# google-research/nerf-from-image

Measured on AMD Instinct MI355X. Metric: rendered rays/sec (128x128, 64+64 samples), higher is better.
Workload: dtype f32 (decoder MLP operands split-fp16 hi+lo, 22 bits; strict fp32: config.value_mlp_exact_fp32)

## Files before the change

### nerf_from_image_amd/csrc/nfi_kernels.hip

```cpp
#include "nfi_device.hpp"
#include "../../include/nfi_hip.h"
#include "nfi_host.hpp"

#include <algorithm>
#include <cstdio>
#include <cstring>

using namespace nfi;

thread_local char nfi_err_buf[256] = "";
extern "C" const char* nfi_last_error(void) { return nfi_err_buf; }
extern "C" int nfi_version(void) { return 100; }


constexpr int kP2tPixels = 256, kP2tPitch = 288;
template <int TEX>
__global__ __launch_bounds__(256) void planes_to_texels_kernel(const float* __restrict__ planes, void* __restrict__ texels,
                                                               int hw) {
  __shared__ __attribute__((aligned(16))) float tile[kC][kP2tPitch];
  const int img = blockIdx.y;
  const int px0 = blockIdx.x * kP2tPixels;
  const float* src = planes + (size_t)img * kC * hw;
  {
    const int c4 = threadIdx.x & 63, r0 = threadIdx.x >> 6;
// ... 166 lines not shown
          w2v[h] = w;
        }
      }
      auto hi = __builtin_amdgcn_cvt_pkrtz(w2v[0], w2v[1]);
      auto lo = __builtin_amdgcn_cvt_pkrtz(w2v[0] - (float)hi[0], w2v[1] - (float)hi[1]);
      v = bits2f(hl == 0 ? __builtin_bit_cast(uint32_t, hi) : __builtin_bit_cast(uint32_t, lo));
    }
    image[i] = v;
  }
}

extern "C" size_t nfi_decoder_image_floats(void) { return (size_t)kImageFloats; }

extern "C" int nfi_decoder_pack(const float* w1, const float* b1, const float* w2, const float* b2, int n_attention,
                                int texel_dtype, float* image, nfi_stream_t stream) {
  REQUIRE(w1 && b1 && w2 && b2 && image, "decoder_pack: null pointer");
  REQUIRE(n_attention >= 0 && n_attention <= NFI_MAX_ATTENTION, "decoder_pack: attention_values must be in [0,14]");
  REQUIRE(texel_dtype >= NFI_TEXEL_F32 && texel_dtype <= NFI_TEXEL_F16, "decoder_pack: bad texel dtype");
  int n_out = n_attention > 0 ? 1 + n_attention : 4;
  hipLaunchKernelGGL(decoder_pack_kernel, dim3((kImageFloats + 255) / 256), dim3(256), 0, (hipStream_t)stream, w1, b1, w2, b2,
                     n_out, texel_dtype, image);
  return check_launch("decoder_pack");
}

__global__ __launch_bounds__(256) void decoder_pack_vd_kernel(const float* __restrict__ w1, const float* __restrict__ b1,
                                                              const float* __restrict__ w2, const float* __restrict__ b2,
                                                              const float* __restrict__ w3, const float* __restrict__ b3,
                                                              int n3, int tex, float* __restrict__ image) {
  const float gain1 = 0.17677669529663687f;
  const float gain2 = 0.125f;
  const float gain3 = 0.17677669529663687f;
  for (int i = threadIdx.x; i < kVdImageFloats; i += blockDim.x) {
    float v = 0.0f;
    if (i < kVdB1F) {
      int k = i - kVdW1F;
      int nt = k & 3, lane = (k >> 2) & 63, s = k >> 8;
      int row = 16 * nt + (lane & 15);
      int ch = feat_channel(tex, s, lane >> 4);
      v = (w1[row * kC + ch] * gain1) * (kLog2e / 3.0f);
    } else if (i < kVdW2) {
      int k = i - kVdB1F;
      int r = k & 3, nt = (k >> 2) & 3, g = k >> 4;
      v = b1[16 * nt + 4 * g + r] * kLog2e;
    } else if (i < kVdB2) {
      int k = i - kVdW2;
      int r = k & 3, lane = (k >> 2) & 63, nt = (k >> 8) & 3, t = k >> 10;
      int row = 16 * t + (lane & 15);
      int hid = 16 * nt + 4 * (lane >> 4) + r;
      if (row < 33) v = (w2[row * kHidden + hid] * gain2) * kLn2;
    } else if (i < kVdW3) {
      int row = i - kVdB2;
      if (row < 33) v = b2[row];
    } else if (i < kVdB3) {
      int k = i - kVdW3;
      int r = k & 3, lane = (k >> 2) & 63, t = k >> 8;
      int out = lane & 15;
      int kk = 16 * t + 4 * (lane >> 4) + r;
      if (out == 0) v = (kk == 0) ? 1.0f : 0.0f;
      else if (out <= n3 && kk >= 1 && kk <= 32) v = (w3[(out - 1) * 32 + (kk - 1)] * gain3) * kLog2e;
    } else {
      int out = i - kVdB3;
      if (out >= 1 && out <= n3) v = b3[out - 1] * kLog2e;
    }
    image[i] = v;
  }
}

extern "C" size_t nfi_decoder_image_floats_viewdir(void) { return (size_t)kVdImageFloats; }

extern "C" int nfi_decoder_pack_viewdir(const float* w1, const float* b1, const float* w2, const float* b2, const float* w3,
                                        const float* b3, int n_attention, int texel_dtype, float* image,
                                        nfi_stream_t stream) {
  REQUIRE(w1 && b1 && w2 && b2 && w3 && b3 && image, "decoder_pack_viewdir: null pointer");
  REQUIRE(n_attention >= 0 && n_attention <= NFI_MAX_ATTENTION, "decoder_pack_viewdir: attention_values must be in [0,14]");
  REQUIRE(texel_dtype >= NFI_TEXEL_F32 && texel_dtype <= NFI_TEXEL_F16, "decoder_pack_viewdir: bad texel dtype");
  static_assert(NFI_RAY_FEATURE_PITCH == kRayFeatPad, "ray feature pitch");
  int n3 = n_attention > 0 ? n_attention : 3;
  hipLaunchKernelGGL(decoder_pack_vd_kernel, dim3(1), dim3(256), 0, (hipStream_t)stream, w1, b1, w2, b2, w3, b3, n3,
                     texel_dtype, image);
  return check_launch("decoder_pack_viewdir");
}

constexpr int kRayBlocks = 256;
__device__ __forceinline__ void block_reduce_keys(uint32_t kmin, uint32_t kmax, uint32_t cnt, uint32_t* reduce) {
  __shared__ uint32_t s_min[4], s_max[4], s_cnt[4];
#pragma unroll
  for (int d = 32; d >= 1; d >>= 1) {
    uint32_t a = (uint32_t)__shfl_xor((int)kmin, d, 64), b = (uint32_t)__shfl_xor((int)kmax, d, 64);
    kmin = a > kmin ? a : kmin;
    kmax = b > kmax ? b : kmax;
    cnt += (uint32_t)__shfl_xor((int)cnt, d, 64);
  }
  int wave = threadIdx.x >> 6;
  if ((threadIdx.x & 63) == 0) { s_min[wave] = kmin; s_max[wave] = kmax; s_cnt[wave] = cnt; }
  __syncthreads();
  if (threadIdx.x == 0) {
    int nw = blockDim.x >> 6;
    for (int w = 1; w < nw; ++w) {
      kmin = s_min[w] > kmin ? s_min[w] : kmin;
      kmax = s_max[w] > kmax ? s_max[w] : kmax;
      cnt += s_cnt[w];
    }
    if (cnt) {
      atomicMax(&reduce[0], kmin);
      atomicMax(&reduce[1], kmax);
      atomicAdd(&reduce[2], cnt);
    }
  }
}

struct RaygenOut {
  float* ro; float* rd;
  float* near_raw; float* far_raw; uint8_t* hit;
  uint32_t* reduce;
  float scene_range;
};

__global__ __launch_bounds__(256) void raygen_kernel(CameraParams cam, int n_scenes, RaygenOut out) {
  const int hw = cam.rows * cam.width;
  const int64_t n = (int64_t)n_scenes * hw;
  uint32_t kmin = 0u, kmax = 0u, cnt = 0u;
  for (int64_t ray = (int64_t)blockIdx.x * blockDim.x + threadIdx.x; ray < n; ray += (int64_t)gridDim.x * blockDim.x) {
    int b = (int)(ray / hw);
    int pix = (int)(ray - (int64_t)b * hw);
    int row = pix / cam.width, col = pix - row * cam.width;
    float o[3], d[3];
    make_ray(cam, b, cam.row0 + row, col, o, d);
    if (out.ro) { out.ro[ray * 3 + 0] = o[0]; out.ro[ray * 3 + 1] = o[1]; out.ro[ray * 3 + 2] = o[2]; }
    if (out.rd) { out.rd[ray * 3 + 0] = d[0]; out.rd[ray * 3 + 1] = d[1]; out.rd[ray * 3 + 2] = d[2]; }
    if (out.near_raw) {
      float near = 0.0f, far = 0.0f;
      const bool hit = slab_test(o, d, out.scene_range, near, far);
      float n2, f2;
      bool hit_wide = slab_test(o, d, out.scene_range * 1.0001f, n2, f2);
      out.near_raw[ray] = near;
      out.far_raw[ray] = far;
      out.hit[ray] = (uint8_t)((hit ? 1 : 0) | (hit_wide ? 2 : 0));
      if (hit) {
        const uint32_t a = ~ordered_key(near), c = ordered_key(far);
        kmin = a > kmin ? a : kmin;
        kmax = c > kmax ? c : kmax;
        ++cnt;
      }
    }
  }
  if (out.near_raw) block_reduce_keys(kmin, kmax, cnt, out.reduce);
}

__global__ __launch_bounds__(256) void slab_kernel(const float* __restrict__ ro, const float* __restrict__ rd, int64_t n,
                                                   float scene_range, float* __restrict__ near_raw,
                                                   float* __restrict__ far_raw, uint8_t* __restrict__ hit_out,
                                                   uint32_t* reduce) {
  uint32_t kmin = 0u, kmax = 0u, cnt = 0u;
  for (int64_t ray = (int64_t)blockIdx.x * blockDim.x + threadIdx.x; ray < n; ray += (int64_t)gridDim.x * blockDim.x) {
    float o[3] = {ro[ray * 3], ro[ray * 3 + 1], ro[ray * 3 + 2]};
    float d[3] = {rd[ray * 3], rd[ray * 3 + 1], rd[ray * 3 + 2]};
    float near = 0.0f, far = 0.0f;
    const bool hit = slab_test(o, d, scene_range, near, far);
    float n2, f2;
    bool hit_wide = slab_test(o, d, scene_range * 1.0001f, n2, f2);
    near_raw[ray] = near;
    far_raw[ray] = far;
    hit_out[ray] = (uint8_t)((hit ? 1 : 0) | (hit_wide ? 2 : 0));
    if (hit) {
      const uint32_t a = ~ordered_key(near), c = ordered_key(far);
      kmin = a > kmin ? a : kmin;
      kmax = c > kmax ? c : kmax;
      ++cnt;
    }
  }
  block_reduce_keys(kmin, kmax, cnt, reduce);
}

__global__ __launch_bounds__(256) void finish_planes_kernel(const float* __restrict__ near_raw,
                                                            const float* __restrict__ far_raw,
                                                            const uint8_t* __restrict__ hit, const uint32_t* __restrict__ reduce,
                                                            int64_t n, float* __restrict__ near_plane,
                                                            float* __restrict__ far_plane) {
  const int64_t ray = (int64_t)blockIdx.x * blockDim.x + threadIdx.x;
  if (ray >= n) return;
  float fill_near = ordered_key_inv(~reduce[0]), fill_far = ordered_key_inv(reduce[1]);
  float a = near_raw[ray], b = far_raw[ray];
  finish_planes((hit[ray] & 1) != 0, fill_near, fill_far, a, b);
  near_plane[ray] = a;
  far_plane[ray] = b;
}

extern "C" int nfi_raygen(const nfi_raygen_args* a, nfi_stream_t stream) {
  REQUIRE(a && a->cam2world && a->ray_origins && a->ray_directions, "raygen: null pointer");
  REQUIRE(a->n_scenes > 0 && a->height > 0 && a->width > 0, "raygen: bad shape");
  CameraParams cam{a->cam2world, a->focal, a->bbox, a->focal ? a->center : nullptr, a->height, a->width, a->normalize, a->height, 0};
  RaygenOut out{a->ray_origins, a->ray_directions, nullptr, nullptr, nullptr, nullptr, 0.0f};
  int64_t n = (int64_t)a->n_scenes * a->height * a->width;
  hipLaunchKernelGGL(raygen_kernel, dim3((unsigned)std::min<int64_t>((n + 255) / 256, kRayBlocks)), dim3(256), 0, (hipStream_t)stream, cam,
                     a->n_scenes, out);
  return check_launch("raygen");
}

extern "C" int nfi_near_far(const nfi_near_far_args* a, nfi_stream_t stream) {
  REQUIRE(a && a->ray_origins && a->ray_directions && a->near_raw && a->far_raw && a->hit && a->reduce,
          "near_far: null pointer");
  REQUIRE(a->n_rays > 0, "near_far: no rays");
  hipStream_t s = (hipStream_t)stream;
  if (hipMemsetAsync(a->reduce, 0, 16, s) != hipSuccess) return fail(NFI_ERR_LAUNCH, "near_far: memset failed");
  unsigned blocks = (unsigned)((a->n_rays + 255) / 256);
  hipLaunchKernelGGL(slab_kernel, dim3(std::min<unsigned>(blocks, kRayBlocks)), dim3(256), 0, s, a->ray_origins, a->ray_directions, a->n_rays,
                     a->scene_range, a->near_raw, a->far_raw, a->hit, a->reduce);
  if (a->near_plane && a->far_plane)
    hipLaunchKernelGGL(finish_planes_kernel, dim3(blocks), dim3(256), 0, s, a->near_raw, a->far_raw, a->hit, a->reduce,
                       a->n_rays, a->near_plane, a->far_plane);
  return check_launch("near_far");
}

__device__ __forceinline__ float stratified_depth(float near, float far, int k, int S, float noise, bool jitter) {
  float t = aten_lerp(near, far, (float)k / (float)S);
  if (jitter) t = t + noise * ((far - near) / (float)S);
  return t;
}

__global__ __launch_bounds__(256) void stratified_kernel(nfi_stratified_args a) {
  const int64_t idx = (int64_t)blockIdx.x * blockDim.x + threadIdx.x;
  const int64_t total = a.n_rays * a.n_samples;
  if (idx >= total) return;
  const int64_t ray = idx / a.n_samples;
  const int k = (int)(idx - ray * a.n_samples);
  float near = a.near_plane[ray], far = a.far_plane[ray];
  float t = stratified_depth(near, far, k, a.n_samples, a.noise ? a.noise[idx] : 0.0f, a.noise != nullptr);
  a.depth[idx] = t;
  if (a.points) {
#pragma unroll
    for (int c = 0; c < 3; ++c) a.points[idx * 3 + c] = a.ray_origins[ray * 3 + c] + a.ray_directions[ray * 3 + c] * t;
  }
}

__global__ __launch_bounds__(256) void points_on_rays_kernel(const float* __restrict__ ro, const float* __restrict__ rd,
                                                             const float* __restrict__ depth, int64_t total, int S,
                                                             float* __restrict__ points) {
  const int64_t idx = (int64_t)blockIdx.x * blockDim.x + threadIdx.x;
  if (idx >= total) return;
  const int64_t ray = idx / S;
  const float t = depth[idx];
#pragma unroll
  for (int c = 0; c < 3; ++c) points[idx * 3 + c] = ro[ray * 3 + c] + rd[ray * 3 + c] * t;
}

extern "C" int nfi_points_on_rays(const float* ray_origins, const float* ray_directions, const float* depth,
                                  int64_t n_rays, int n_samples, float* points, nfi_stream_t stream) {
  REQUIRE(ray_origins && ray_directions && depth && points, "points_on_rays: null pointer");
  REQUIRE(n_rays > 0 && n_samples > 0, "points_on_rays: bad shape");
  int64_t total = n_rays * n_samples;
  hipLaunchKernelGGL(points_on_rays_kernel, dim3((unsigned)((total + 255) / 256)), dim3(256), 0, (hipStream_t)stream,
                     ray_origins, ray_directions, depth, total, n_samples, points);
  return check_launch("points_on_rays");
}
// ... 721 lines not shown
    }
  }
  if (a.n_extra > 0 && a.extra_map) {
    wave_lds_fence();
#pragma unroll
    for (int j = 0; j < NS; ++j) {
      int e = j * 64 + lane;
      if (e < n) slab.cdf[e] = w[j];
    }
    wave_lds_fence();
    float we[NS];
#pragma unroll
    for (int j = 0; j < NS; ++j) { int e = j * 64 + lane; we[j] = e < n ? slab.cdf[rank[j]] : 0.0f; }
    for (int c = 0; c < a.n_extra; ++c) {
      float acc = 0.0f;
#pragma unroll
      for (int j = 0; j < NS; ++j) {
        int e = j * 64 + lane;
        if (e < na) acc += we[j] * a.extra_a[((size_t)ray * na + e) * a.n_extra + c];
        else if (e < n) acc += we[j] * a.extra_b[((size_t)ray * nb + (e - na)) * a.n_extra + c];
      }
      acc = wave_sum(acc);
      if (lane == 0) a.extra_map[ray * a.n_extra + c] = acc;
    }
  }
}

extern "C" int nfi_composite_fwd(const nfi_composite_args* a, nfi_stream_t stream) {
  REQUIRE(a && a->ray_directions && a->depth_a && a->sigma_a && a->rgb_a && a->rgb_map && a->depth_map && a->mask,
          "composite: null pointer");
  REQUIRE(a->n_rays > 0 && a->n_a > 0 && a->n_b >= 0 && a->n_a + a->n_b <= NFI_MAX_SAMPLES_SINGLE_PASS,
          "composite: need 1 <= n_a + n_b <= 512");
  REQUIRE(a->n_b == 0 || (a->n_a <= NFI_MAX_SAMPLES && a->n_b <= NFI_MAX_SAMPLES), "composite: merged lists hold at most 128 samples each");
  REQUIRE(a->n_b == 0 || (a->depth_b && a->sigma_b && a->rgb_b), "composite: list b missing");
  REQUIRE(a->n_extra == 0 || (a->extra_a && (a->n_b == 0 || a->extra_b)), "composite: extra attribute missing");
  const dim3 grid((unsigned)((a->n_rays + 3) / 4));
  if (a->n_a + a->n_b <= 128) hipLaunchKernelGGL(composite_kernel<2>, grid, dim3(256), 0, (hipStream_t)stream, *a);
  else if (a->n_a + a->n_b <= 256) hipLaunchKernelGGL(composite_kernel<4>, grid, dim3(256), 0, (hipStream_t)stream, *a);
  else hipLaunchKernelGGL(composite_kernel<8>, grid, dim3(256), 0, (hipStream_t)stream, *a);
  return check_launch("composite_fwd");
}

#include "nfi_backward_rays.inc"
#include "nfi_regulariser.inc"
#include "nfi_neighbours.inc"
#include "nfi_handoff.inc"
#include "nfi_pnp.inc"

struct RenderKernelParams {
  int n_scenes, hw, S;
  int fine, white;
  float scene_range;
  const float* ro; const float* rd; const float* near_raw; const float* far_raw; const uint8_t* hit;
  const uint32_t* reduce;
  uint32_t* counter;
  int width;
  int tile_order;
  int xcd_blocks;
  uint32_t* xcd_counter;
  int xcd_block_shift;
  int fetch_batch;
  const void* texels; int res; int layout;
  const float* image; int A; const float* att;
  int use_sdf; const float* beta; const float* alpha;
  const float* noise_c; const float* noise_f; int64_t noise_f_stride;
  float* rgb; float* depth; float* mask;
  float* near_plane; float* far_plane;
  float* t_coarse; float* sigma_coarse; float* rgb_coarse;
  float* t_fine; float* sigma_fine; float* rgb_fine;
  float* t_sorted; float* weights; int32_t* perm;
  int skip_missed;
  unsigned long long* prof;
  const float* xray;
  float term_eps;
  float* semantics;
  float* coords;
  float* normals;
  unsigned long long* clock_probe;
  FastDiv div_hw, div_bps, div_bw;
  int tap_stride;
  int stash;
};

struct ClockProbe {
  unsigned long long c0 = 0, r0 = 0;
  bool on = false;
  __device__ __forceinline__ void start(const RenderKernelParams& k) {
    on = k.clock_probe && blockIdx.x == 0 && threadIdx.x == 0;
    if (on) { c0 = __builtin_readcyclecounter(); r0 = __builtin_amdgcn_s_memrealtime(); }
  }
  __device__ __forceinline__ void stop(const RenderKernelParams& k) const {
    if (on) {
      k.clock_probe[0] = __builtin_readcyclecounter() - c0;
      k.clock_probe[1] = __builtin_amdgcn_s_memrealtime() - r0;
    }
  }
};

__device__ __forceinline__ float uniform_f32(float v) {
  return bits2f((uint32_t)__builtin_amdgcn_readfirstlane((int)f2bits(v)));
}

struct RayInputs {
  float ox, oy, oz, dx, dy, dz, near, far, noise, u;
  uint32_t hit;
};

struct RayQueue {
  const RenderKernelParams& k;
  int lane;
  uint32_t n_rays, xcd, bsh, bw, bps, n_blocks, q_cur, pos_next, pos_end, batch;
  bool dry;
  __device__ __forceinline__ RayQueue(const RenderKernelParams& kk, int l) : k(kk), lane(l) {
    n_rays = (uint32_t)k.n_scenes * (uint32_t)k.hw;
    xcd = k.xcd_blocks ? (__builtin_amdgcn_s_getreg(6164) & 7u) : 0u;
    bsh = (uint32_t)k.xcd_block_shift;
    bw = (uint32_t)k.width >> bsh;
    bps = bw * (((uint32_t)k.hw / (uint32_t)k.width) >> bsh);
    n_blocks = bps * (uint32_t)k.n_scenes;
    q_cur = xcd; pos_next = 0; pos_end = 0; dry = false;
    batch = (uint32_t)k.fetch_batch;
  }
  __device__ __forceinline__ uint32_t ray_at(uint32_t q, uint32_t pos) const {
    const uint32_t b = (pos >> (2 * bsh)) * 8u + q;
    const uint32_t in = pos & ((1u << (2 * bsh)) - 1u), scene = fastdiv(b, k.div_bps), bb = b - scene * bps;
    const uint32_t by = fastdiv(bb, k.div_bw), bx = bb - by * bw;
    const uint32_t st = in >> 6, sty = st >> (bsh - 3), stx = st & ((1u << (bsh - 3)) - 1u);
    const uint32_t y = (by << bsh) + (sty << 3) + ((in >> 3) & 7u), x = (bx << bsh) + (stx << 3) + (in & 7u);
    return scene * (uint32_t)k.hw + y * (uint32_t)k.width + x;
  }
  __device__ __forceinline__ uint32_t fetch() {
    if (!k.xcd_blocks) {
      uint32_t p = 0;
      if (lane == 0) p = atomicAdd(k.counter, 1u);
      return (uint32_t)__builtin_amdgcn_readfirstlane((int)p);
    }
    if (pos_next == pos_end && !dry) {
      dry = true;
      for (uint32_t i = 0; i < 8; ++i) {
        uint32_t base = 0;
        if (lane == 0) base = atomicAdd(k.xcd_counter + q_cur * 16, batch);
        base = (uint32_t)__builtin_amdgcn_readfirstlane((int)base);
        if ((base >> (2 * bsh)) * 8u + q_cur < n_blocks) { pos_next = base; pos_end = base + batch; dry = false; break; }
        q_cur = (q_cur + 1) & 7u;
      }
    }
    if (dry) return n_rays;
    return ray_at(q_cur, pos_next++);
  }
};

constexpr int kRenderPlain = 0, kRenderTaps = 1, kRenderProf = 2, kRenderTerm = 3, kRenderExtra = 4, kRenderNormals = 5;
constexpr int kSemPitch = 2 * 64 + 4;
constexpr int kSemPitchWide = 2 * 128 + 8;
extern __shared__ __attribute__((aligned(16))) float nfi_dyn_lds[];

typedef __attribute__((address_space(3))) float lds_float;

template <int NS, class Slab>
__device__ __forceinline__ void composite_coords(const Slab& slab, const float (&w)[NS], int n, int lane, float ox, float oy,
                                                 float oz, float dx, float dy, float dz, float* out3) {
  float cx = 0.0f, cy = 0.0f, cz = 0.0f;
#pragma unroll
  for (int j = 0; j < NS; ++j) {
    const int e = j * 64 + lane;
    if (e < n) {
      const float t = slab.srt[0][e];
      cx += w[j] * (ox + dx * t); cy += w[j] * (oy + dy * t); cz += w[j] * (oz + dz * t);
    }
  }
  cx = wave_sum(cx); cy = wave_sum(cy); cz = wave_sum(cz);
  if (lane == 0) { out3[0] = cx; out3[1] = cy; out3[2] = cz; }
}

template <int TEX, bool ATT, int OCC, int MODE, int PREC, bool VD = false>
__global__ __launch_bounds__(256, OCC) void render_fwd_kernel(RenderKernelParams k) {
  constexpr bool TAPS = MODE == kRenderTaps, PROF = MODE == kRenderProf, TERM = MODE == kRenderTerm;
  constexpr bool EXTRA = MODE == kRenderExtra || MODE == kRenderNormals, NRM = MODE == kRenderNormals;
  constexpr int SEMP = (EXTRA && ATT) ? kSemPitch : 0;
  constexpr int kImg = VD ? kVdImageFloats : kLdsImageFloats;
  __shared__ __attribute__((aligned(16))) float lds[kImg];
  __shared__ __attribute__((aligned(16))) float vfs[4][64];
  __shared__ WaveSlab slabs[4];
  if constexpr (NRM) stage_normal_operands(nfi_dyn_lds, k.image, VD ? kVdW1F : kW1F, VD ? kVdW2 : kW2F);
  ClockProbe clock;
  clock.start(k);
  if (PREC == 1) {
    for (int i = threadIdx.x; i < kB1F; i += blockDim.x) lds[i] = k.image[kW1H + i];
    for (int i = kB1F + threadIdx.x; i < kLdsImageFloats; i += blockDim.x) lds[i] = k.image[i];
  } else {
    for (int i = threadIdx.x; i < kImg; i += blockDim.x) lds[i] = k.image[i];
  }
  __syncthreads();
  const int lane = lane_id();
  const int wave = threadIdx.x >> 6;
  WaveSlab& slab = slabs[wave];
  float* vf = vfs[wave];
  const int S = k.S;
  const bool valid = lane < S;
  const float fill_near = ordered_key_inv(~k.reduce[0]), fill_far = ordered_key_inv(k.reduce[1]);
  const float bg = k.white ? 1.0f : 0.0f;
  const size_t tb = TEX == 0 ? 128 : 64;
  const uint32_t n_rays = (uint32_t)k.n_scenes * (uint32_t)k.hw;
  const uint32_t tiles_x = (uint32_t)k.width >> 3;
  auto ray_of = [&](uint32_t pos) -> uint32_t {
    if (k.xcd_blocks || !k.tile_order) return pos;
    const uint32_t scene = pos / (uint32_t)k.hw, p = pos - scene * (uint32_t)k.hw;
    const uint32_t tile = p >> 6, in = p & 63u;
    const uint32_t ty = tile / tiles_x, tx = tile - ty * tiles_x;
    return scene * (uint32_t)k.hw + ((ty << 3) + (in >> 3)) * (uint32_t)k.width + (tx << 3) + (in & 7u);
  };

  FieldParams P = make_field_params(k.texels, k.res, TEX, k.A, k.use_sdf, k.beta, k.alpha, lds, kImg, k.layout);
  P.vf = vf;
  P.w1t = nfi_dyn_lds; P.w2r0 = nfi_dyn_lds + kW1TFloats;
  int cur_scene = -1;

  float* semT = nullptr;
  if constexpr (SEMP > 0) {
    if (k.semantics) {
      semT = nfi_dyn_lds + (NRM ? kNrmLdsFloats : 0) + wave * (k.A * kSemPitch);
      for (int i = lane; i < k.A * kSemPitch; i += 64) ((lds_float*)semT)[i] = 0.0f;
      wave_lds_fence();
    }
  }

  auto load_inputs = [&](uint32_t ray, RayInputs& in) {
    const size_t r3 = (size_t)ray * 3;
    in.hit = k.hit[ray];
    in.ox = k.ro[r3]; in.oy = k.ro[r3 + 1]; in.oz = k.ro[r3 + 2];
    in.dx = k.rd[r3]; in.dy = k.rd[r3 + 1]; in.dz = k.rd[r3 + 2];
    in.near = k.near_raw[ray]; in.far = k.far_raw[ray];
    in.noise = (k.noise_c && valid) ? k.noise_c[(size_t)ray * S + lane] : 0.0f;
    in.u = (k.fine && valid) ? k.noise_f[(size_t)ray * k.noise_f_stride + lane] : 0.0f;
  };

  RayQueue queue(k, lane);
  auto fetch = [&]() -> uint32_t { return queue.fetch(); };
  uint32_t cur = fetch(), nxt = fetch(), fly = 0;
  RayInputs in, pre;
  unsigned long long pc[12] = {0, 0, 0, 0, 0, 0, 0, 0, 0, 0, 0, 0};
  unsigned long long tk0 = PROF ? __builtin_readcyclecounter() : 0;
  if (cur < n_rays) load_inputs(ray_of(cur), in);
  while (cur < n_rays) {
    if (nxt < n_rays) load_inputs(ray_of(nxt), pre);
    const uint32_t ray = ray_of(cur);
    const uint32_t hitb = in.hit;
    float out_r = bg, out_g = bg, out_b = bg, out_d = 0.0f, out_m = 0.0f;
    if (k.skip_missed && !(hitb & 2)) {
      if constexpr (EXTRA) {
        if (k.coords && lane < 3) k.coords[(size_t)ray * 3 + lane] = 0.0f;
        if (k.semantics && lane < k.A) k.semantics[(size_t)ray * k.A + lane] = 0.0f;
        if (NRM && lane < 3) k.normals[(size_t)ray * 3 + lane] = bg;
      }
      if constexpr (TAPS) {
        if (k.stash && valid) {
          const size_t zs = (size_t)ray * (size_t)k.tap_stride + lane;
          k.t_coarse[zs] = 0.0f; k.sigma_coarse[zs] = 0.0f;
          float* q = k.rgb_coarse + zs * 3; q[0] = 0.0f; q[1] = 0.0f; q[2] = 0.0f;
          if (k.fine) {
            k.t_fine[zs] = 0.0f; k.sigma_fine[zs] = 0.0f;
            q = k.rgb_fine + zs * 3; q[0] = 0.0f; q[1] = 0.0f; q[2] = 0.0f;
          }
        }
      }
    } else {
      unsigned long long t0 = PROF ? __builtin_readcyclecounter() : 0;
      const int scene = (int)fastdiv(ray, k.div_hw);
      if (scene != cur_scene) {
        cur_scene = scene;
        const char* tex_scene = reinterpret_cast<const char*>(k.texels) + (size_t)scene * 3 * k.res * k.res * tb;
        P.rsrc = __builtin_amdgcn_make_buffer_rsrc(const_cast<char*>(tex_scene), 0, (int)P.scene_bytes, 0x00020000);
        wave_lds_fence();
        {
          int c = lane & 3, row = lane >> 2;
          float v = 0.0f;
          if (k.att && c < 3 && row >= 1 && row <= k.A) v = k.att[((size_t)scene * k.A + (row - 1)) * 3 + c];
          vf[lane] = v;
        }
        wave_lds_fence();
      }
      const float ox = in.ox, oy = in.oy, oz = in.oz, dx = in.dx, dy = in.dy, dz = in.dz;
      float near = in.near, far = in.far;
      finish_planes((hitb & 1) != 0, fill_near, fill_far, near, far);
      const float dnorm = norm3(dx, dy, dz);
      const size_t rs = (size_t)ray * (size_t)k.tap_stride;

      float tc = 0.0f;
      if (valid) tc = stratified_depth(near, far, lane, S, in.noise, k.noise_c != nullptr);
      MergeIn c;
      float ncx = 0.0f, ncy = 0.0f, ncz = 0.0f, nfx = 0.0f, nfy = 0.0f, nfz = 0.0f;
      unsigned long long t1 = PROF ? __builtin_readcyclecounter() : 0;
      {
        SampleOut q = field_wave<TEX, ATT, true, PREC, VD, SEMP, NRM>(P, k.scene_range, lane, ox + dx * tc, oy + dy * tc, oz + dz * tc,
                                                                      valid, semT, nullptr, &slab.srt[0][0], PROF ? pc : nullptr,
                                                                      k.xray, (int)ray);
        c.t = tc; c.sigma = q.sigma; c.r = q.r; c.g = q.g; c.b = q.b;
        if constexpr (NRM) { ncx = q.nx; ncy = q.ny; ncz = q.nz; }
      }
      int n = S;
      int rank_c = lane, rank_f = 0;
      unsigned long long t2 = PROF ? __builtin_readcyclecounter() : 0, t3 = t2, t4 = t2, t5 = t2;
      if (k.fine) {
        ResampleTaps rt;
        float tf = resample_ray(slab, c.sigma, tc, S, dnorm, in.u, lane, TERM ? &rt : nullptr);
        MergeIn f;
        if (PROF) { asm volatile("" :: "v"(tf)); t3 = __builtin_readcyclecounter(); }
        if constexpr (TERM) {
          const uint64_t dm = __ballot(valid && rt.T < k.term_eps);
          float t_dead = INFINITY;
          if (dm) t_dead = bits2f((uint32_t)__builtin_amdgcn_readlane((int)f2bits(tc), (int)__builtin_ctzll(dm)));
          const bool live = valid && tf <= t_dead;
          const uint64_t lm = __ballot(live);
          const int nl = __builtin_popcountll(lm);
          const int nb = __builtin_popcountll(lm & ((1ull << lane) - 1ull));
          const int pos = live ? nb : nl + (lane - nb);
          wave_lds_fence();
          slab.cdf[pos] = tf;
          wave_lds_fence();
          tf = slab.cdf[lane];
          wave_lds_fence();
          const bool vl = lane < nl;
          SampleOut q = field_wave<TEX, ATT, true, PREC, VD>(P, k.scene_range, lane, ox + dx * tf, oy + dy * tf, oz + dz * tf, vl,
                                                             nullptr, nullptr, &slab.srt[0][0], nullptr, k.xray, (int)ray);
          f.t = tf; f.sigma = vl ? q.sigma : 0.0f; f.r = vl ? q.r : 0.0f; f.g = vl ? q.g : 0.0f; f.b = vl ? q.b : 0.0f;
        } else {
          SampleOut q = field_wave<TEX, ATT, true, PREC, VD, SEMP, NRM>(P, k.scene_range, lane, ox + dx * tf, oy + dy * tf, oz + dz * tf,
// ... 77 lines not shown
        pc[4] += t1 - t0; pc[5] += t2 - t1; pc[6] += t3 - t2; pc[7] += t4 - t3; pc[8] += t5 - t4; pc[9] += t6 - t5; pc[10] += 1;
      }
    }
    fly = fetch();
    if (lane == 0) {
      k.rgb[(size_t)ray * 3] = out_r; k.rgb[(size_t)ray * 3 + 1] = out_g; k.rgb[(size_t)ray * 3 + 2] = out_b;
      k.depth[ray] = out_d; k.mask[ray] = out_m;
    }
    in = pre;
    cur = nxt;
    nxt = fly;
  }
  if (PROF && k.prof && lane == 0) {
    pc[11] = __builtin_readcyclecounter() - tk0;
    for (int i = 0; i < 12; ++i) atomicAdd(k.prof + i, pc[i]);
  }
  clock.stop(k);
}

#ifdef NFI_SINGLE_KERNEL
#ifndef NFI_SINGLE_MODE
#define NFI_SINGLE_MODE 0
#endif
template __global__ void render_fwd_kernel<NFI_SINGLE_KERNEL, true, NFI_RENDER_OCC, NFI_SINGLE_MODE, 1>(RenderKernelParams);
#endif
#if !defined(NFI_SINGLE_KERNEL) || defined(NFI_SINGLE_WIDE)
template <int TEX, bool ATT, int MODE, int PREC, bool VD = false, int OCC = NFI_RENDER_OCC>
__global__ __launch_bounds__(256, OCC) void render_fwd_wide_kernel(RenderKernelParams k) {
  constexpr bool TAPS = MODE == kRenderTaps, TERM = MODE == kRenderTerm;
  constexpr bool EXTRA = MODE == kRenderExtra || MODE == kRenderNormals, NRM = MODE == kRenderNormals;
  constexpr int SEMP = (EXTRA && ATT) ? -kSemPitchWide : 0;
  constexpr int kImg = VD ? kVdImageFloats : kLdsImageFloats;
  __shared__ __attribute__((aligned(16))) float lds[kImg];
  __shared__ __attribute__((aligned(16))) float vfs[4][64];
  __shared__ WaveSlabWide slabs[4];
  if constexpr (NRM) stage_normal_operands(nfi_dyn_lds, k.image, VD ? kVdW1F : kW1F, VD ? kVdW2 : kW2F);
  ClockProbe clock;
  clock.start(k);
  if (PREC == 1) {
    for (int i = threadIdx.x; i < kB1F; i += blockDim.x) lds[i] = k.image[kW1H + i];
    for (int i = kB1F + threadIdx.x; i < kLdsImageFloats; i += blockDim.x) lds[i] = k.image[i];
  } else {
    for (int i = threadIdx.x; i < kImg; i += blockDim.x) lds[i] = k.image[i];
  }
  __syncthreads();
  const int lane = lane_id();
  const int wave = threadIdx.x >> 6;
  WaveSlabWide& slab = slabs[wave];
  float* vf = vfs[wave];
  const int S = k.S;
  const float fill_near = ordered_key_inv(~k.reduce[0]), fill_far = ordered_key_inv(k.reduce[1]);
  const float bg = k.white ? 1.0f : 0.0f;
  const size_t tb = TEX == 0 ? 128 : 64;
  const uint32_t n_rays = (uint32_t)k.n_scenes * (uint32_t)k.hw;
  const uint32_t tiles_x = (uint32_t)k.width >> 3;
  auto ray_of = [&](uint32_t pos) -> uint32_t {
    if (k.xcd_blocks || !k.tile_order) return pos;
    const uint32_t scene = pos / (uint32_t)k.hw, p = pos - scene * (uint32_t)k.hw;
    const uint32_t tile = p >> 6, in = p & 63u;
    const uint32_t ty = tile / tiles_x, tx = tile - ty * tiles_x;
    return scene * (uint32_t)k.hw + ((ty << 3) + (in >> 3)) * (uint32_t)k.width + (tx << 3) + (in & 7u);
  };
  FieldParams P = make_field_params(k.texels, k.res, TEX, k.A, k.use_sdf, k.beta, k.alpha, lds, kImg, k.layout);
  P.vf = vf;
  P.w1t = nfi_dyn_lds; P.w2r0 = nfi_dyn_lds + kW1TFloats;
  int cur_scene = -1;
  typedef __attribute__((address_space(3))) unsigned short lds_u16;
  float* semT = nullptr;
  if constexpr (SEMP != 0) {
    if (k.semantics) {
      semT = reinterpret_cast<float*>(reinterpret_cast<unsigned short*>(nfi_dyn_lds + (NRM ? kNrmLdsFloats : 0)) +
                                      wave * (k.A * kSemPitchWide));
      for (int i = lane; i < k.A * kSemPitchWide / 2; i += 64) ((lds_float*)semT)[i] = 0.0f;
      wave_lds_fence();
    }
  }
  auto sem_col = [&](int c) -> float* {
    return semT ? reinterpret_cast<float*>(reinterpret_cast<unsigned short*>(semT) + c) : nullptr;
  };
  RayQueue queue(k, lane);
  uint32_t cur = queue.fetch(), nxt = 0;
  while (cur < n_rays) {
    nxt = queue.fetch();
    const uint32_t ray = ray_of(cur);
    const uint32_t hitb = k.hit[ray];
    if (k.skip_missed && !(hitb & 2)) {
      if (lane == 0) {
        k.rgb[(size_t)ray * 3] = bg; k.rgb[(size_t)ray * 3 + 1] = bg; k.rgb[(size_t)ray * 3 + 2] = bg;
        k.depth[ray] = 0.0f; k.mask[ray] = 0.0f;
      }
      if constexpr (EXTRA) {
        if (k.coords && lane < 3) k.coords[(size_t)ray * 3 + lane] = 0.0f;
        if (k.semantics && lane < k.A) k.semantics[(size_t)ray * k.A + lane] = 0.0f;
        if (NRM && lane < 3) k.normals[(size_t)ray * 3 + lane] = bg;
      }
      if constexpr (TAPS) {
        if (k.stash) {
#pragma unroll
          for (int j = 0; j < 2; ++j) {
            if (j * 64 + lane < S) {
              const size_t zs = (size_t)ray * (size_t)k.tap_stride + j * 64 + lane;
              k.t_coarse[zs] = 0.0f; k.sigma_coarse[zs] = 0.0f;
              float* q = k.rgb_coarse + zs * 3; q[0] = 0.0f; q[1] = 0.0f; q[2] = 0.0f;
              if (k.fine) {
                k.t_fine[zs] = 0.0f; k.sigma_fine[zs] = 0.0f;
                q = k.rgb_fine + zs * 3; q[0] = 0.0f; q[1] = 0.0f; q[2] = 0.0f;
              }
            }
          }
        }
      }
    } else {
      const int scene = (int)fastdiv(ray, k.div_hw);
      if (scene != cur_scene) {
        cur_scene = scene;
        const char* tex_scene = reinterpret_cast<const char*>(k.texels) + (size_t)scene * 3 * k.res * k.res * tb;
        P.rsrc = __builtin_amdgcn_make_buffer_rsrc(const_cast<char*>(tex_scene), 0, (int)P.scene_bytes, 0x00020000);
        wave_lds_fence();
        {
          int c = lane & 3, row = lane >> 2;
          float v = 0.0f;
          if (k.att && c < 3 && row >= 1 && row <= k.A) v = k.att[((size_t)scene * k.A + (row - 1)) * 3 + c];
          vf[lane] = v;
        }
        wave_lds_fence();
      }
      const size_t r3 = (size_t)ray * 3;
      const float ox = k.ro[r3], oy = k.ro[r3 + 1], oz = k.ro[r3 + 2];
      const float dx = k.rd[r3], dy = k.rd[r3 + 1], dz = k.rd[r3 + 2];
      float near = k.near_raw[ray], far = k.far_raw[ray];
      finish_planes((hitb & 1) != 0, fill_near, fill_far, near, far);
      const float dnorm = norm3(dx, dy, dz);
      const size_t rs = (size_t)ray * S;
      const size_t ts = (size_t)ray * (size_t)k.tap_stride;
      float* stage = &slab.srt[0][0];

      float tc[2], sc[2], rc[2], gc[2], bc[2];
      bool val[2];
#pragma unroll
      for (int j = 0; j < 2; ++j) {
        const int e = j * 64 + lane;
        val[j] = e < S;
        const float nz = (k.noise_c && val[j]) ? k.noise_c[rs + e] : 0.0f;
        tc[j] = val[j] ? stratified_depth(near, far, e, S, nz, k.noise_c != nullptr) : 0.0f;
      }
      float nrm[4][3];
#pragma unroll
      for (int j = 0; j < 4; ++j) nrm[j][0] = nrm[j][1] = nrm[j][2] = 0.0f;
#pragma unroll
      for (int j = 0; j < 2; ++j) {
        SampleOut q = field_wave<TEX, ATT, true, PREC, VD, SEMP, NRM>(P, k.scene_range, lane, ox + dx * tc[j], oy + dy * tc[j],
                                                                      oz + dz * tc[j], val[j], sem_col(j * 64), nullptr,
                                                                      stage, nullptr, k.xray, (int)ray);
        sc[j] = q.sigma; rc[j] = q.r; gc[j] = q.g; bc[j] = q.b;
        if constexpr (NRM) { nrm[j][0] = q.nx; nrm[j][1] = q.ny; nrm[j][2] = q.nz; }
      }
      int n = S;
      float dep[4], sig[4], cr[4], cg[4], cb[4];
      int eidx[4], rank[4];
#pragma unroll
      for (int j = 0; j < 2; ++j) {
        dep[j] = tc[j]; sig[j] = sc[j]; cr[j] = rc[j]; cg[j] = gc[j]; cb[j] = bc[j];
        eidx[j] = val[j] ? j * 64 + lane : 0x7fffffff;
        dep[2 + j] = sig[2 + j] = cr[2 + j] = cg[2 + j] = cb[2 + j] = 0.0f;
        eidx[2 + j] = 0x7fffffff;
        rank[j] = j * 64 + lane; rank[2 + j] = 0;
// ... 106 lines not shown
          if (k.near_plane) k.near_plane[ray] = near;
          if (k.far_plane) k.far_plane[ray] = far;
        }
#pragma unroll
        for (int j = 0; j < 2; ++j) {
          if (val[j]) {
            const size_t i = ts + j * 64 + lane;
            if (k.t_coarse) k.t_coarse[i] = tc[j];
            if (k.sigma_coarse) k.sigma_coarse[i] = sc[j];
            if (k.rgb_coarse) { float* o3 = k.rgb_coarse + i * 3; o3[0] = rc[j]; o3[1] = gc[j]; o3[2] = bc[j]; }
            if (k.perm) {
              k.perm[(size_t)ray * n + rank[j]] = j * 64 + lane;
              if (k.fine) k.perm[(size_t)ray * n + rank[2 + j]] = S + j * 64 + lane;
            }
          }
        }
#pragma unroll
        for (int j = 0; j < 4; ++j) {
          int e = j * 64 + lane;
          if (e < n) {
            if (k.weights) k.weights[(size_t)ray * n + e] = w[j];
            if (k.t_sorted) k.t_sorted[(size_t)ray * n + e] = slab.srt[0][e];
          }
        }
      }
      wave_lds_fence();
    }
    cur = nxt;
  }
  clock.stop(k);
}

#endif
#ifdef NFI_SINGLE_WIDE
template __global__ void render_fwd_wide_kernel<NFI_SINGLE_KERNEL, true, NFI_SINGLE_MODE, 1, false, NFI_RENDER_OCC>(RenderKernelParams);
#endif
#ifndef NFI_SINGLE_KERNEL
struct __attribute__((aligned(16))) WaveSlabLong {
  float srt[5][NFI_MAX_SAMPLES_SINGLE_PASS];
  float stage[16 * 36];
};

template <int TEX, bool ATT, int PREC, bool VD = false>
__global__ __launch_bounds__(256, NFI_RENDER_OCC) void render_fwd_long_kernel(RenderKernelParams k) {
  constexpr int kImg = VD ? kVdImageFloats : kLdsImageFloats;
  constexpr int NS = NFI_MAX_SAMPLES_SINGLE_PASS / 64;
  __shared__ __attribute__((aligned(16))) float lds[kImg];
  __shared__ __attribute__((aligned(16))) float vfs[4][64];
  __shared__ WaveSlabLong slabs[4];
  ClockProbe clock;
  clock.start(k);
  if (PREC == 1) {
    for (int i = threadIdx.x; i < kB1F; i += blockDim.x) lds[i] = k.image[kW1H + i];
    for (int i = kB1F + threadIdx.x; i < kLdsImageFloats; i += blockDim.x) lds[i] = k.image[i];
  } else {
    for (int i = threadIdx.x; i < kImg; i += blockDim.x) lds[i] = k.image[i];
  }
  __syncthreads();
  const int lane = lane_id();
  const int wave = threadIdx.x >> 6;
  WaveSlabLong& slab = slabs[wave];
  float* vf = vfs[wave];
  const int S = k.S;
  const int slots = (S + 63) >> 6;
  const float fill_near = ordered_key_inv(~k.reduce[0]), fill_far = ordered_key_inv(k.reduce[1]);
  const float bg = k.white ? 1.0f : 0.0f;
  const size_t tb = TEX == 0 ? 128 : 64;
  const uint32_t n_rays = (uint32_t)k.n_scenes * (uint32_t)k.hw;
  const uint32_t tiles_x = (uint32_t)k.width >> 3;
  auto ray_of = [&](uint32_t pos) -> uint32_t {
    if (k.xcd_blocks || !k.tile_order) return pos;
    const uint32_t scene = pos / (uint32_t)k.hw, p = pos - scene * (uint32_t)k.hw;
    const uint32_t tile = p >> 6, in = p & 63u;
    const uint32_t ty = tile / tiles_x, tx = tile - ty * tiles_x;
    return scene * (uint32_t)k.hw + ((ty << 3) + (in >> 3)) * (uint32_t)k.width + (tx << 3) + (in & 7u);
  };
  FieldParams P = make_field_params(k.texels, k.res, TEX, k.A, k.use_sdf, k.beta, k.alpha, lds, kImg, k.layout);
  P.vf = vf;
  int cur_scene = -1;
  RayQueue queue(k, lane);
  uint32_t cur = queue.fetch(), nxt = 0;
  while (cur < n_rays) {
    nxt = queue.fetch();
    const uint32_t ray = ray_of(cur);
    const uint32_t hitb = k.hit[ray];
    const size_t ts = (size_t)ray * (size_t)k.tap_stride;
    if (k.skip_missed && !(hitb & 2)) {
      if (lane == 0) {
        k.rgb[(size_t)ray * 3] = bg; k.rgb[(size_t)ray * 3 + 1] = bg; k.rgb[(size_t)ray * 3 + 2] = bg;
        k.depth[ray] = 0.0f; k.mask[ray] = 0.0f;
      }
      if (k.stash) {
        for (int e = lane; e < S; e += 64) {
          k.t_coarse[ts + e] = 0.0f; k.sigma_coarse[ts + e] = 0.0f;
          float* q = k.rgb_coarse + (ts + e) * 3; q[0] = 0.0f; q[1] = 0.0f; q[2] = 0.0f;
        }
      }
    } else {
      const int scene = (int)fastdiv(ray, k.div_hw);
      if (scene != cur_scene) {
        cur_scene = scene;
        const char* tex_scene = reinterpret_cast<const char*>(k.texels) + (size_t)scene * 3 * k.res * k.res * tb;
        P.rsrc = __builtin_amdgcn_make_buffer_rsrc(const_cast<char*>(tex_scene), 0, (int)P.scene_bytes, 0x00020000);
        wave_lds_fence();
        {
          int c = lane & 3, row = lane >> 2;
          float v = 0.0f;
          if (k.att && c < 3 && row >= 1 && row <= k.A) v = k.att[((size_t)scene * k.A + (row - 1)) * 3 + c];
          vf[lane] = v;
        }
        wave_lds_fence();
      }
      const size_t r3 = (size_t)ray * 3;
      const float ox = k.ro[r3], oy = k.ro[r3 + 1], oz = k.ro[r3 + 2];
      const float dx = k.rd[r3], dy = k.rd[r3 + 1], dz = k.rd[r3 + 2];
      float near = k.near_raw[ray], far = k.far_raw[ray];
      finish_planes((hitb & 1) != 0, fill_near, fill_far, near, far);
      const float dnorm = norm3(dx, dy, dz);
      const size_t rs = (size_t)ray * S;
#pragma unroll 1
      for (int j = 0; j < slots; ++j) {
        const int e = j * 64 + lane;
        const bool val = e < S;
        const float nz = (k.noise_c && val) ? k.noise_c[rs + e] : 0.0f;
        const float t = val ? stratified_depth(near, far, e, S, nz, k.noise_c != nullptr) : 0.0f;
        SampleOut q = field_wave<TEX, ATT, true, PREC, VD>(P, k.scene_range, lane, ox + dx * t, oy + dy * t, oz + dz * t, val,
                                                           nullptr, nullptr, slab.stage, nullptr, k.xray, (int)ray);
        if (val) {
          slab.srt[0][e] = t; slab.srt[1][e] = q.sigma; slab.srt[2][e] = q.r; slab.srt[3][e] = q.g; slab.srt[4][e] = q.b;
          if (k.t_coarse) k.t_coarse[ts + e] = t;
          if (k.sigma_coarse) k.sigma_coarse[ts + e] = q.sigma;
          if (k.rgb_coarse) { float* o3 = k.rgb_coarse + (ts + e) * 3; o3[0] = q.r; o3[1] = q.g; o3[2] = q.b; }
        }
      }
      wave_lds_fence();
      float w[NS];
      CompositeOut o = composite_slab<NS>(slab, S, dnorm, k.white, lane, w);
      if (lane == 0) {
        k.rgb[(size_t)ray * 3] = o.r; k.rgb[(size_t)ray * 3 + 1] = o.g; k.rgb[(size_t)ray * 3 + 2] = o.b;
        k.depth[ray] = o.depth; k.mask[ray] = o.mask;
        if (k.near_plane) k.near_plane[ray] = near;
        if (k.far_plane) k.far_plane[ray] = far;
      }
      if (k.weights || k.t_sorted || k.perm) {
#pragma unroll
        for (int j = 0; j < NS; ++j) {
          const int e = j * 64 + lane;
          if (e < S) {
            if (k.weights) k.weights[rs + e] = w[j];
            if (k.t_sorted) k.t_sorted[rs + e] = slab.srt[0][e];
            if (k.perm) k.perm[rs + e] = e;
          }
        }
      }
      wave_lds_fence();
    }
    cur = nxt;
  }
  clock.stop(k);
}

extern "C" size_t nfi_render_workspace_bytes(int64_t n_rays) {
  size_t n = (size_t)n_rays;
  return n * 8 * sizeof(float) + ((n + 63) & ~(size_t)63) + 64 + 8 * 64;
}

struct RenderWorkspace { uint32_t* reduce; uint32_t* xcd_counter; float* ro; float* rd; float* near_raw; float* far_raw; uint8_t* hit; int64_t n; };

static int render_carve(const nfi_render_args* a, RenderWorkspace& w) {
  REQUIRE(a && a->cam2world && a->workspace, "render: null pointer");
  REQUIRE(a->n_scenes > 0 && a->height > 0 && a->width > 0, "render: bad image shape");
  const int64_t n = (int64_t)a->n_scenes * a->height * a->width;
  if (a->workspace_bytes < nfi_render_workspace_bytes(n)) return fail(NFI_ERR_WORKSPACE_TOO_SMALL, "render: workspace too small");
  float* ws = reinterpret_cast<float*>(a->workspace);
  constexpr int kRays0 = 16 + 128;
  w.n = n;
  w.reduce = reinterpret_cast<uint32_t*>(ws);
  w.xcd_counter = reinterpret_cast<uint32_t*>(ws + 16);
  w.ro = a->ray_origins ? a->ray_origins : ws + kRays0;
  w.rd = a->ray_directions ? a->ray_directions : ws + kRays0 + 3 * n;
  w.near_raw = ws + kRays0 + 6 * n;
  w.far_raw = ws + kRays0 + 7 * n;
  w.hit = a->hit ? a->hit : reinterpret_cast<uint8_t*>(ws + kRays0 + 8 * n);
  return NFI_OK;
}

static int render_setup(const nfi_render_args* a, const RenderWorkspace& w, hipStream_t s) {
  if (hipMemsetAsync(w.reduce, 0, 64 + 8 * 64, s) != hipSuccess) return fail(NFI_ERR_LAUNCH, "render: memset failed");
  const int full_h = a->full_height > 0 ? a->full_height : a->height;
  REQUIRE(a->row_offset >= 0 && a->row_offset + a->height <= full_h, "render: row window outside the image");
  CameraParams cam{a->cam2world, a->focal, a->bbox, a->focal ? a->center : nullptr, full_h, a->width, 1, a->height, a->row_offset};
  RaygenOut rout{w.ro, w.rd, w.near_raw, w.far_raw, w.hit, w.reduce, a->scene_range};
  hipLaunchKernelGGL(raygen_kernel, dim3((unsigned)std::min<int64_t>((w.n + 255) / 256, kRayBlocks)), dim3(256), 0, s, cam, a->n_scenes, rout);
  return NFI_OK;
}

extern "C" int nfi_render_setup(const nfi_render_args* a, nfi_stream_t stream) {
  RenderWorkspace w;
  int rc = render_carve(a, w);
  if (rc) return rc;
  rc = render_setup(a, w, (hipStream_t)stream);
  if (rc) return rc;
  return check_launch("render_setup");
}

extern "C" int nfi_render_fwd(const nfi_render_args* a, nfi_stream_t stream) {
  REQUIRE(a && a->cam2world && a->rgb && a->depth && a->mask && a->workspace, "render: null pointer");
  REQUIRE(a->n_scenes > 0 && a->height > 0 && a->width > 0, "render: bad image shape");
  REQUIRE(a->n_samples >= 4 && a->n_samples <= (a->fine_sampling ? NFI_MAX_SAMPLES : NFI_MAX_SAMPLES_SINGLE_PASS),
          "render: n_samples must be in [4,128] per pass with fine sampling, [4,512] for a single pass");
  REQUIRE(a->n_samples <= 64 || !a->profile_cycles, "render: the cycle profile exists for n_samples <= 64 only");
  REQUIRE(a->n_samples <= NFI_MAX_SAMPLES || !(a->semantics || a->coords || a->normals),
          "render: semantics / coords / normals maps exist for n_samples <= 128");
  REQUIRE(!a->fine_sampling || a->noise_fine, "render: fine sampling needs u (noise_fine)");
  REQUIRE(!a->semantics || a->n_attention > 0, "render: composited semantics need attention values (A > 0)");
  int rc = check_field_common(a->texels, a->plane_res, a->texel_dtype, a->decoder_image, a->n_attention,
                               a->attention_values, a->use_sdf, a->beta, a->alpha, a->texel_layout);
  if (rc) return rc;
  RenderWorkspace w;
  rc = render_carve(a, w);
  if (rc) return rc;
  const int64_t n = w.n;
  hipStream_t s = (hipStream_t)stream;
  uint32_t* reduce = w.reduce;
  uint32_t* xcd_counter = w.xcd_counter;
  float *ro = w.ro, *rd = w.rd, *near_raw = w.near_raw, *far_raw = w.far_raw;
  uint8_t* hit = w.hit;
  REQUIRE(!(a->rays_ready && (a->ray_origins || a->ray_directions || a->hit || a->stash_t)),
          "render: rays_ready needs the ray set-up in the workspace (no ray_origins / ray_directions / hit taps, no stash)");
  if (!a->rays_ready) {
    rc = render_setup(a, w, s);
    if (rc) return rc;
  }

  const bool stash = a->stash_t || a->stash_sigma || a->stash_rgb;
  REQUIRE(!stash || (a->stash_t && a->stash_sigma && a->stash_rgb), "render: the training stash needs stash_t, stash_sigma and stash_rgb");
  REQUIRE(!stash || !(a->t_coarse || a->sigma_coarse || a->rgb_coarse || a->t_fine || a->sigma_fine || a->rgb_fine),
          "render: the training stash and the per-sample debug taps are mutually exclusive");
  const bool debug_tap = a->t_coarse || a->sigma_coarse || a->rgb_coarse || a->t_fine || a->sigma_fine || a->rgb_fine ||
                         a->t_sorted || a->weights || a->perm || a->near_plane || a->far_plane;
  const bool any_tap = debug_tap || stash;
  RenderKernelParams k;
  memset(&k, 0, sizeof(k));
  k.n_scenes = a->n_scenes; k.hw = a->height * a->width; k.S = a->n_samples;
  k.fine = a->fine_sampling; k.white = a->white_background; k.scene_range = a->scene_range;
  k.ro = ro; k.rd = rd; k.near_raw = near_raw; k.far_raw = far_raw; k.hit = hit; k.reduce = reduce;
  k.texels = a->texels; k.res = a->plane_res; k.layout = a->texel_layout; k.image = a->decoder_image; k.A = a->n_attention; k.att = a->attention_values;
  k.use_sdf = a->use_sdf; k.beta = a->beta; k.alpha = a->alpha;
  k.noise_c = a->noise_coarse; k.noise_f = a->noise_fine; k.noise_f_stride = a->noise_fine_row_stride;
  k.rgb = a->rgb; k.depth = a->depth; k.mask = a->mask;
  k.near_plane = a->near_plane; k.far_plane = a->far_plane;
  k.t_coarse = a->t_coarse; k.sigma_coarse = a->sigma_coarse; k.rgb_coarse = a->rgb_coarse;
  k.t_fine = a->t_fine; k.sigma_fine = a->sigma_fine; k.rgb_fine = a->rgb_fine;
  k.tap_stride = a->n_samples;
  if (stash) {
    k.tap_stride = (a->fine_sampling ? 2 : 1) * a->n_samples; k.stash = 1;
    k.t_coarse = a->stash_t; k.sigma_coarse = a->stash_sigma; k.rgb_coarse = a->stash_rgb;
    if (a->fine_sampling) {
      k.t_fine = a->stash_t + a->n_samples;
      k.sigma_fine = a->stash_sigma + a->n_samples;
      k.rgb_fine = a->stash_rgb + 3 * (size_t)a->n_samples;
    }
  }
  k.t_sorted = a->t_sorted; k.weights = a->weights; k.perm = a->perm;
  k.skip_missed = (a->skip_missed_rays && !debug_tap) ? 1 : 0;

  k.counter = reduce + 3;
  k.width = a->width;
  {
    k.fetch_batch = 2;
    const int both = a->width | a->height;
    k.xcd_block_shift = (both & 31) == 0 ? 5 : ((both & 15) == 0 ? 4 : 3);
    const int side = 1 << k.xcd_block_shift;
    k.xcd_blocks = (((a->tuning >> 4) & 1) == 0 && (a->width % side == 0) && (a->height % side == 0)) ? 1 : 0;
    const uint32_t bw = (uint32_t)a->width >> k.xcd_block_shift, bh = (uint32_t)a->height >> k.xcd_block_shift;
    k.div_hw = make_fastdiv((uint32_t)k.hw);
// ... 135 lines not shown
```

Baseline: 145.3 million.

## Replace setup memset and global atomics with per-block slots and a finish kernel

The render setup no longer memsets the reduce/counter area. Raygen blocks now write per-block min/max/count partials to workspace slots, and a single-block finish kernel reduces those slots and zeroes the XCD counters. The raygen grid also grows from at most 256 to at most 1024 blocks. This removes a memset launch and the contention on global atomics, at the cost of an extra small kernel launch and a little more workspace. A compile-time wave timing probe is also added but is off by default.

```diff
diff --git a/nerf_from_image_amd/csrc/nfi_kernels.hip b/nerf_from_image_amd/csrc/nfi_kernels.hip
--- a/nerf_from_image_amd/csrc/nfi_kernels.hip
+++ b/nerf_from_image_amd/csrc/nfi_kernels.hip
@@ -272,7 +272,8 @@
 }
 
 constexpr int kRayBlocks = 256;
-__device__ __forceinline__ void block_reduce_keys(uint32_t kmin, uint32_t kmax, uint32_t cnt, uint32_t* reduce) {
+constexpr int kSetupSlots = 1024;
+__device__ __forceinline__ void block_reduce_keys(uint32_t& kmin, uint32_t& kmax, uint32_t& cnt) {
   __shared__ uint32_t s_min[4], s_max[4], s_cnt[4];
 #pragma unroll
   for (int d = 32; d >= 1; d >>= 1) {
@@ -291,18 +292,13 @@
       kmax = s_max[w] > kmax ? s_max[w] : kmax;
       cnt += s_cnt[w];
     }
-    if (cnt) {
-      atomicMax(&reduce[0], kmin);
-      atomicMax(&reduce[1], kmax);
-      atomicAdd(&reduce[2], cnt);
-    }
   }
 }
 
 struct RaygenOut {
   float* ro; float* rd;
   float* near_raw; float* far_raw; uint8_t* hit;
-  uint32_t* reduce;
+  uint4* slots;
   float scene_range;
 };
 
@@ -334,7 +330,24 @@
       }
     }
   }
-  if (out.near_raw) block_reduce_keys(kmin, kmax, cnt, out.reduce);
+  if (out.near_raw) {
+    block_reduce_keys(kmin, kmax, cnt);
+    if (threadIdx.x == 0) out.slots[blockIdx.x] = make_uint4(kmin, kmax, cnt, 0u);
+  }
+}
+
+__global__ __launch_bounds__(256) void setup_finish_kernel(const uint4* __restrict__ slots, int n_slots, uint32_t* reduce,
+                                                           uint32_t* xcd_counter) {
+  uint32_t kmin = 0u, kmax = 0u, cnt = 0u;
+  for (int i = threadIdx.x; i < n_slots; i += blockDim.x) {
+    const uint4 s = slots[i];
+    kmin = s.x > kmin ? s.x : kmin;
+    kmax = s.y > kmax ? s.y : kmax;
+    cnt += s.z;
+  }
+  block_reduce_keys(kmin, kmax, cnt);
+  if (threadIdx.x == 0) { reduce[0] = kmin; reduce[1] = kmax; reduce[2] = cnt; reduce[3] = 0u; }
+  if (threadIdx.x < 8) xcd_counter[threadIdx.x * 16] = 0u;
 }
 
 __global__ __launch_bounds__(256) void slab_kernel(const float* __restrict__ ro, const float* __restrict__ rd, int64_t n,
@@ -359,7 +372,12 @@
       ++cnt;
     }
   }
-  block_reduce_keys(kmin, kmax, cnt, reduce);
+  block_reduce_keys(kmin, kmax, cnt);
+  if (threadIdx.x == 0 && cnt) {
+    atomicMax(&reduce[0], kmin);
+    atomicMax(&reduce[1], kmax);
+    atomicAdd(&reduce[2], cnt);
+  }
 }
 
 __global__ __launch_bounds__(256) void finish_planes_kernel(const float* __restrict__ near_raw,
@@ -1247,6 +1265,7 @@
   int stash;
 };
 
+#ifndef NFI_WAVE_PROBE
 struct ClockProbe {
   unsigned long long c0 = 0, r0 = 0;
   bool on = false;
@@ -1254,6 +1273,7 @@
     on = k.clock_probe && blockIdx.x == 0 && threadIdx.x == 0;
     if (on) { c0 = __builtin_readcyclecounter(); r0 = __builtin_amdgcn_s_memrealtime(); }
   }
+  __device__ __forceinline__ void ray(bool) {}
   __device__ __forceinline__ void stop(const RenderKernelParams& k) const {
     if (on) {
       k.clock_probe[0] = __builtin_readcyclecounter() - c0;
@@ -1261,6 +1281,33 @@
     }
   }
 };
+#else
+constexpr int kWaveProbe = 8;
+struct ClockProbe {
+  unsigned long long t0 = 0, t_first = 0, t_dry = 0;
+  uint32_t n = 0, n_after = 0;
+  bool on = false;
+  __device__ __forceinline__ void start(const RenderKernelParams& k) {
+    on = k.clock_probe != nullptr;
+    t0 = __builtin_amdgcn_s_memrealtime();
+  }
+  __device__ __forceinline__ void ray(bool dry) {
+    const unsigned long long t = __builtin_amdgcn_s_memrealtime();
+    if (n == 0) t_first = t;
+    if (dry && t_dry == 0) t_dry = t;
+    n_after += (dry ? 1u : 0u);
+    ++n;
+  }
+  __device__ __forceinline__ void stop(const RenderKernelParams& k) {
+    const unsigned long long t = __builtin_amdgcn_s_memrealtime();
+    if (on && (threadIdx.x & 63) == 0) {
+      unsigned long long* o = k.clock_probe + kWaveProbe * (size_t)(4 * blockIdx.x + (threadIdx.x >> 6));
+      o[0] = t0; o[1] = t_first; o[2] = t_dry ? t_dry : t; o[3] = t; o[4] = n; o[5] = n_after;
+      o[6] = __builtin_amdgcn_s_getreg(6164) & 7u; o[7] = 0;
+    }
+  }
+};
+#endif
 
 __device__ __forceinline__ float uniform_f32(float v) {
   return bits2f((uint32_t)__builtin_amdgcn_readfirstlane((int)f2bits(v)));
@@ -1408,6 +1455,7 @@
   unsigned long long tk0 = PROF ? __builtin_readcyclecounter() : 0;
   if (cur < n_rays) load_inputs(ray_of(cur), in);
   while (cur < n_rays) {
+    clock.ray(queue.dry);
     if (nxt < n_rays) load_inputs(ray_of(nxt), pre);
     const uint32_t ray = ray_of(cur);
     const uint32_t hitb = in.hit;
@@ -1651,6 +1699,7 @@
   uint32_t cur = queue.fetch(), nxt = 0;
   while (cur < n_rays) {
     nxt = queue.fetch();
+    clock.ray(queue.dry);
     const uint32_t ray = ray_of(cur);
     const uint32_t hitb = k.hit[ray];
     if (k.skip_missed && !(hitb & 2)) {
@@ -1923,6 +1972,7 @@
   uint32_t cur = queue.fetch(), nxt = 0;
   while (cur < n_rays) {
     nxt = queue.fetch();
+    clock.ray(queue.dry);
     const uint32_t ray = ray_of(cur);
     const uint32_t hitb = k.hit[ray];
     const size_t ts = (size_t)ray * (size_t)k.tap_stride;
@@ -2001,12 +2051,14 @@
   clock.stop(k);
 }
 
+static unsigned setup_blocks(int64_t n) { return (unsigned)std::min<int64_t>((n + 255) / 256, kSetupSlots); }
+
 extern "C" size_t nfi_render_workspace_bytes(int64_t n_rays) {
   size_t n = (size_t)n_rays;
-  return n * 8 * sizeof(float) + ((n + 63) & ~(size_t)63) + 64 + 8 * 64;
-}
-
-struct RenderWorkspace { uint32_t* reduce; uint32_t* xcd_counter; float* ro; float* rd; float* near_raw; float* far_raw; uint8_t* hit; int64_t n; };
+  return n * 8 * sizeof(float) + ((n + 63) & ~(size_t)63) + 64 + 8 * 64 + (size_t)setup_blocks(n_rays) * sizeof(uint4);
+}
+
+struct RenderWorkspace { uint32_t* reduce; uint32_t* xcd_counter; float* ro; float* rd; float* near_raw; float* far_raw; uint8_t* hit; uint4* slots; int64_t n; };
 
 static int render_carve(const nfi_render_args* a, RenderWorkspace& w) {
   REQUIRE(a && a->cam2world && a->workspace, "render: null pointer");
@@ -2023,16 +2075,18 @@
   w.near_raw = ws + kRays0 + 6 * n;
   w.far_raw = ws + kRays0 + 7 * n;
   w.hit = a->hit ? a->hit : reinterpret_cast<uint8_t*>(ws + kRays0 + 8 * n);
+  w.slots = reinterpret_cast<uint4*>(reinterpret_cast<uint8_t*>(ws + kRays0 + 8 * n) + ((n + 63) & ~(int64_t)63));
   return NFI_OK;
 }
 
 static int render_setup(const nfi_render_args* a, const RenderWorkspace& w, hipStream_t s) {
-  if (hipMemsetAsync(w.reduce, 0, 64 + 8 * 64, s) != hipSuccess) return fail(NFI_ERR_LAUNCH, "render: memset failed");
   const int full_h = a->full_height > 0 ? a->full_height : a->height;
   REQUIRE(a->row_offset >= 0 && a->row_offset + a->height <= full_h, "render: row window outside the image");
   CameraParams cam{a->cam2world, a->focal, a->bbox, a->focal ? a->center : nullptr, full_h, a->width, 1, a->height, a->row_offset};
-  RaygenOut rout{w.ro, w.rd, w.near_raw, w.far_raw, w.hit, w.reduce, a->scene_range};
-  hipLaunchKernelGGL(raygen_kernel, dim3((unsigned)std::min<int64_t>((w.n + 255) / 256, kRayBlocks)), dim3(256), 0, s, cam, a->n_scenes, rout);
+  RaygenOut rout{w.ro, w.rd, w.near_raw, w.far_raw, w.hit, w.slots, a->scene_range};
+  const unsigned blocks = setup_blocks(w.n);
+  hipLaunchKernelGGL(raygen_kernel, dim3(blocks), dim3(256), 0, s, cam, a->n_scenes, rout);
+  hipLaunchKernelGGL(setup_finish_kernel, dim3(1), dim3(256), 0, s, w.slots, (int)blocks, w.reduce, w.xcd_counter);
   return NFI_OK;
 }
 
```

After: 146.6 million, median of 6. No clear change (+0.9%).
